# atneit/SCA-LDPC

Measured on AMD Instinct MI355X. Metric: edge_message_updates_per_s, higher is better.
Workload: dtype f32; 1 GPU; hqc128 H=[Hin|I] N=17669 W=50 R=4000 E=204000, batch 4096/GPU, 50 fixed iters, min_sum; batch_per_gpu=4096, iters=50, tile_group=0

## Files before the change

### sca-ldpc_amd/csrc/scaldpc_bp.hip

```cpp
#include "scaldpc_common.h"
#include "scaldpc_bp_sched.h"
#include "scaldpc_mc_law.h"
#include "scaldpc_trials.h"

#include <algorithm>
#include <cfloat>
#include <cmath>
#include <cstdlib>
#include <cstring>
#include <mutex>
#include <unordered_map>
#include <vector>

typedef unsigned long long u64;

using namespace scaldpc;

#include "scaldpc_bp_kernels.h"
#include "scaldpc_bp_ref64.h"

namespace scaldpc {
int launch_mc_hqc_outcome64(const McHqcLaw64 &law, unsigned long long *synd, double *plane, int R, int batch, int T, long first,
                            unsigned k0, unsigned k1, int *acc_flips, int *acc_cost, uint8_t *out_outcome, hipStream_t s);
int launch_gather_prior64(const double *src, int cols, const int *ids, double *dst, int T2, hipStream_t s);
// ... 604 lines not shown
    const dim3 grid(h->row_bk.blk[h->row_bk.nb], G), block(256);
    const bool test = ft && !first;
    if (method != SCALDPC_BP_MIN_SUM) {
        with_cap<16, 32, 64>(h->max_row_deg, [&](auto cap) {
            if (test)
                hipLaunchKernelGGL((k_check_tanh<cap, false, true, SharedPrior>), grid, block, 0, s, h->d_row_list, msg0, scr0, synd_g,
                                   done_g, skip_done, h->m, h->E, h->d_col_idx, h->d_prior, *ft);
            else
                with_first_prior(h, first, sp, [&](auto fst, auto P, auto prior) {
                    hipLaunchKernelGGL((k_check_tanh<cap, fst, false, decltype(P)>), grid, block, 0, s, h->d_row_list, msg0, scr0,
                                       synd_g, done_g, skip_done, h->m, h->E, h->d_col_idx, prior, FusedTest{});
                });
        });
    } else if (rec_form(h, method) && !first) {
        float *const rec0 = h->d_rec + (size_t)tile0 * rec_tile_floats(h->m);
        u64 *const mask0 = h->d_mask + (size_t)tile0 * h->E;
        const FusedTest ft0 = test ? *ft : FusedTest{};
        const float *const cprior = sp ? nullptr : h->d_prior;
        with_cap<16, 32, 64>(h->max_row_deg, [&](auto cap) {
            with_bool(boot, [&](auto bt) {
                with_bool(test, [&](auto par) {
                    hipLaunchKernelGGL((k_check_minsum_rec<cap, bt, par>), grid, block, 0, s, h->d_row_list, msg0, synd_g, done_g,
                                       skip_done, h->m, h->E, alpha, h->d_col_idx, rec0, mask0, h->d_csr_pos, cprior, ft0, stl);
                });
            });
        });
    } else if (h->max_row_deg <= ROW_CAP) {
        with_cap<16, 32, 64>(h->max_row_deg, [&](auto cap) {
            if (test)
                hipLaunchKernelGGL((k_check_minsum_x<cap, false, true, SharedPrior>), grid, block, 0, s, h->d_row_list, msg0, synd_g,
                                   done_g, skip_done, h->m, h->E, alpha, h->d_col_idx, h->d_prior, *ft);
            else
                with_first_prior(h, first, sp, [&](auto fst, auto P, auto prior) {
                    hipLaunchKernelGGL((k_check_minsum_x<cap, fst, false, decltype(P)>), grid, block, 0, s, h->d_row_list, msg0,
                                       synd_g, done_g, skip_done, h->m, h->E, alpha, h->d_col_idx, prior, FusedTest{});
                });
        });
    } else {
        with_first_prior(h, first, sp, [&](auto fst, auto P, auto prior) {
            hipLaunchKernelGGL((k_check_minsum<fst, decltype(P)>), dim3((h->m + 3) / 4, G), block, 0, s, h->d_row_ptr, msg0, synd_g,
                               done_g, skip_done, h->m, h->E, alpha, h->d_col_idx, prior);
        });
    }
    LAUNCH_CHECK();
    return 0;
}

bool first_fusable(const scaldpc_bp *h, int method)
{
    return h->kn.first_fused && fused_init(h, method) && h->E > 0 && h->max_row_deg <= 64 && h->max_col_deg <= 64 &&
           !h->hg_var.has_generic;
}

int ensure_first_table(scaldpc_bp *h, int method, float alpha1, hipStream_t s)
{
    if (h->first_valid && h->first_method == method && h->first_alpha == alpha1) return 0;
    h->first_valid = false;
    SC_TRY(grow(h->d_first_tab, (size_t)h->E + 128));
    Buf<u64> zero;
    Buf<float> tmp;
    SC_TRY(tmp.ensure((size_t)h->E));
    SC_TRY(zero.ensure((size_t)h->m + 1));
    hipError_t e = hipMemsetAsync(zero, 0, sizeof(u64) * ((size_t)h->m + 1), s);
    if (e == hipSuccess) e = hipMemsetAsync(h->d_first_tab, 0, sizeof(int2) * h->d_first_tab.cap(), s);
    if (e == hipSuccess) {
        with_method(method, [&](auto M) {
            hipLaunchKernelGGL((k_el_check<M, true, SharedPrior>), dim3((h->m + 3) / 4, 1), dim3(256), 0, s, h->d_row_ptr, h->d_col_idx,
                               h->d_prior, tmp, zero, zero + h->m, 0, h->m, h->E, alpha1, (const u64 *)nullptr, (int *)nullptr);
        });
        hipLaunchKernelGGL(k_first_tab, dim3((unsigned)((h->E + 255) / 256)), dim3(256), 0, s, h->d_csc_list, tmp, h->d_row_ptr, h->m,
                           h->E, h->d_first_tab);
        e = hipGetLastError();
    }
    if (e == hipSuccess) e = hipStreamSynchronize(s);
    if (e != hipSuccess) return fail(SCALDPC_EHIP, "first-message table: %s", hipGetErrorString(e));
    h->first_valid = true;
    h->first_method = method;
    h->first_alpha = alpha1;
    return 0;
}

int launch_var(scaldpc_bp *h, int G, float *post_g, u64 *hard_g, const u64 *done_g, int skip_done, int write_out,
               hipStream_t s, int tile0 = 0, const u64 *first_synd = nullptr, bool rec = false, bool light = false,
               const SoftPrior *sp = nullptr, bool final_pass = false, const Settle &stl = Settle{})
{
    float *const msg0 = h->d_msg + (size_t)tile0 * h->E * TW;
    float *const scr0 = h->d_scratch ? h->d_scratch + (size_t)tile0 * h->E * TW : nullptr;
    const int nblk = h->var_bk.blk[h->var_bk.nb];
    if (first_synd) {
        const int nrec = 4 * nblk;
        const dim3 grid2((unsigned)((nrec + 7) / 8), G);
        with_cap<16, 32, 64>(h->max_col_deg, [&](auto cap) {
            hipLaunchKernelGGL((k_var_first<cap>), grid2, dim3(256), 0, s, h->d_var_meta, h->d_csc_list, h->d_prior, msg0, post_g,
                               hard_g, done_g, skip_done, h->n, h->E, write_out, (const int2 *)h->d_first_tab, first_synd, h->m, nrec);
        });
    } else if (rec) {
        const int n1 = (h->var_bk.nb > 0 && h->var_bk.maxd[0] == 1) ? h->var_bk.blk[1] : 0;
        const bool slim = light && !write_out && n1 > 0 && n1 < nblk;
        const int nb_launch = slim ? nblk - n1 : nblk;
        const bool xm = G == 2 || G == 4 || G == 8;
        const dim3 gridr((unsigned)(xm ? (nb_launch + 7) / 8 * 8 : nb_launch), G);
        const int blk0 = slim && !h->var_reversed ? n1 : 0, xmap = xm ? nb_launch : 0;
        with_cap<16, 32>(h->max_col_deg, [&](auto cap) {
            with_prior(h, sp, [&](auto P, auto prior) {
                with_bool(final_pass && write_out, [&](auto fin) {
                    hipLaunchKernelGGL((k_var_rec<cap, decltype(P), fin>), gridr, dim3(256), 0, s, h->d_var_meta, h->d_var_rows,
                                       h->d_csc_list, h->d_csc_row, prior, msg0, h->d_rec + (size_t)tile0 * rec_tile_floats(h->m),
                                       h->d_mask + (size_t)tile0 * h->E, post_g, hard_g, done_g, skip_done, h->n, h->m, h->E,
                                       write_out, blk0, xmap, stl);
                });
            });
        });
    } else {
        with_cap<16, 32, 64>(h->max_col_deg, [&](auto cap) {
            with_prior(h, sp, [&](auto P, auto prior) {
                hipLaunchKernelGGL((k_var<cap, decltype(P)>), dim3(nblk, G), dim3(256), 0, s, h->d_var_meta, h->d_csc_list, prior, msg0,
                                   scr0, post_g, hard_g, done_g, skip_done, h->n, h->E, write_out);
            });
        });
    }
    LAUNCH_CHECK();
    return 0;
}

int launch_el_check(scaldpc_bp *h, int method, float alpha, int nb, const u64 *synd_g, const u64 *done_g,
                    int skip_done, hipStream_t s, bool first, const u64 *hard_g = nullptr, int *unsat_prev = nullptr,
                    const SoftPrior *sp = nullptr)
{
    with_method(method, [&](auto M) {
        with_first_prior(h, first, sp, [&](auto fst, auto P, auto prior) {
            hipLaunchKernelGGL((k_el_check<M, fst, decltype(P)>), dim3((h->m + 3) / 4, nb), dim3(256), 0, s, h->d_row_ptr,
                               h->d_col_idx, prior, h->d_emsg, synd_g, done_g, skip_done, h->m, h->E, alpha, hard_g, unsat_prev);
        });
    });
    LAUNCH_CHECK();
    return 0;
}

int launch_el_var(scaldpc_bp *h, int nb, float *post_g, u64 *hard_g, u64 *done_g, int skip_done, int write_out,
                  hipStream_t s, const int *unsat_prev = nullptr, int it_prev = 0, u64 *conv_g = nullptr,
                  int *iters_g = nullptr, int *remaining_prev = nullptr, const SoftPrior *sp = nullptr)
{
    const unsigned gx = (unsigned)(((h->el_waves + 3) / 4 + 7) / 8 * 8);
    with_prior(h, sp, [&](auto P, auto prior) {
        hipLaunchKernelGGL((k_el_var<decltype(P)>), dim3(gx, nb), dim3(256), 0, s, (const int2 *)h->d_el_slots, h->d_el_slot_col,
                           h->el_waves, prior, h->d_emsg, post_g, hard_g, done_g, skip_done, h->E, write_out, unsat_prev, it_prev,
                           conv_g, iters_g, remaining_prev);
    });
    LAUNCH_CHECK();
    return 0;
}

int launch_syndrome(const scaldpc_bp *h, const u64 *x, u64 *synd, int T, hipStream_t s)
{
    hipLaunchKernelGGL(k_parity<false>, dim3(parity_blocks(h->m), T), dim3(256), 0, s, h->d_row_ptr, h->d_col_idx, x, h->m, h->n,
                       synd, (u64 *)nullptr, (const u64 *)nullptr);
    LAUNCH_CHECK();
    return 0;
}

size_t small_lds_bytes(const scaldpc_bp *h) { return (size_t)2 * h->E * sizeof(float) + (size_t)2 * h->n + h->m + 64; }
size_t small_lds(const scaldpc_bp *h)
{
    const size_t lds = small_lds_bytes(h);
    const bool fits = h->E > 0 && lds <= 60 * 1024;
    return fits && h->kn.path != Knobs::STREAM && h->kn.path != Knobs::EDGE ? lds : 0;
}

template <bool PLANES>
int launch_small(scaldpc_bp *h, size_t lds, int method, int batch, const void *in, int input_kind, int max_iter, float alpha,
                 bool early, void *bits, float *llr, int *iters, void *conv, hipStream_t s, const SoftPrior *sp = nullptr)
{
    with_method(method, [&](auto M) {
        auto launch = [&](auto P, auto prior) {
            hipLaunchKernelGGL((k_bp_small<M, PLANES, decltype(P)>), dim3(batch), dim3(256), lds, s, h->d_row_ptr, h->d_col_idx,
                               h->d_col_ptr, h->d_csc_edge, prior, h->m, h->n, (int)h->E, in, input_kind, max_iter, alpha,
                               early ? 1 : 0, bits, llr, iters, conv);
        };
        with_prior(h, sp, launch);
    });
    LAUNCH_CHECK();
    return 0;
}

float alpha_for(float alpha, int it)
{
    return alpha == 0.0f ? (float)(1.0 - std::pow(2.0, -1.0 * it)) : alpha;
}

struct TileState {
    const u64 *synd;
    u64 *hard, *done, *conv, *unsat;
// ... 55 lines not shown
constexpr int MAX_LANES = SCHED_MAX_LANES;
int fixed_lanes(const scaldpc_bp *h, int g)
{
    if (h->E == 0) return 1;
    return lanes_of(h->kn.split, g);
}
int ensure_lanes(scaldpc_bp *h, int nl)
{
    for (int k = 1; k < nl; k++)
        if (!h->aux_stream[k]) {
            int dev = 0;
            SC_TRY(stream_acquire(&h->aux_stream[k], &dev));
            SC_HIP(hipEventCreateWithFlags(&h->ev_join[k], hipEventDisableTiming));
            SC_HIP(hipEventCreateWithFlags(&h->ev_phase[k], hipEventDisableTiming));
        }
    if (nl > 1 && !h->ev_join[0]) SC_HIP(hipEventCreateWithFlags(&h->ev_join[0], hipEventDisableTiming));
    return 0;
}
struct Lanes {
    scaldpc_bp *h;
    hipStream_t s;
    int n = 1;
    bool open = false;
    Lanes(scaldpc_bp *h_, hipStream_t s_) : h(h_), s(s_) {}
    Lanes(const Lanes &) = delete;
    Lanes &operator=(const Lanes &) = delete;
    ~Lanes() { if (open) (void)join(); }
    hipStream_t operator[](int k) const { return k ? h->aux_stream[k] : s; }
    int fork(int nl)
    {
        n = nl;
        open = nl > 1;
        if (!open) return 0;
        SC_HIP(hipEventRecord(h->ev_join[0], s));
        for (int k = 1; k < n; k++) SC_HIP(hipStreamWaitEvent(h->aux_stream[k], h->ev_join[0], 0));
        return 0;
    }
    int join()
    {
        for (int k = 1; k < n; k++) {
            SC_HIP(hipEventRecord(h->ev_join[k], h->aux_stream[k]));
            SC_HIP(hipStreamWaitEvent(s, h->ev_join[k], 0));
        }
        open = false;
        return 0;
    }
};


struct SettlePlan {
    unsigned *words = nullptr;
    int first_test = 0, horizon = 0;
};
int iterate_tiles(scaldpc_bp *h, Lanes &lanes, const TileState &st, int g0, int g, int max_iter, int method, float alpha,
                  bool early, int defer_after, bool *deferred, int real_codewords, PollState &ps, int chain,
                  const SettlePlan &sl = SettlePlan{})
{
    const hipStream_t s = lanes.s;
    const int skip = early ? 1 : 0;
    const int nl = fixed_lanes(h, g);
    SC_TRY(ensure_lanes(h, nl));
    int gs[MAX_LANES], t0[MAX_LANES];
    deal_tiles(g, nl, gs, t0);
    const int pw = parity_waves(h);
    const bool fused = fused_init(h, method);
    const bool soft = st.pprior != nullptr;
    if (h->E && !fused) {
        const SoftPrior spv = soft ? soft_prior(h, st, g0) : SoftPrior{};
        with_prior(h, soft ? &spv : nullptr, [&](auto P, auto prior) {
            hipLaunchKernelGGL((k_init_msg<decltype(P)>), dim3((unsigned)((h->E + 3) / 4), g), dim3(256), 0, s, h->d_col_idx,
                               h->d_msg.get(), h->E, prior);
        });
        LAUNCH_CHECK();
    }
    int *rem = h->d_remaining;
    if (early) SC_TRY(next_remaining_row(h, s, &rem, lanes.open));
    if (!(chain & 1)) SC_TRY(lanes.fork(nl));
    const bool first_fuse = first_fusable(h, method) && !soft;
    if (first_fuse) SC_TRY(ensure_first_table(h, method, alpha_for(alpha, 1), s));
    const bool ride = early && h->kn.fuse_test && check_can_test(h, method) && pw >= FT_WORDS;
    bool verdict_pending[MAX_LANES] = {};
    const bool recf = rec_form(h, method);
    bool rec_booted[MAX_LANES] = {};
    bool set_phase = true;
    const bool tracked = sl.words && recf && !early;
    const int K = tracked ? sl.horizon : 0, last_test = K ? K : max_iter;
    if (K) h->settle_saved += (long)nl * settle_launches_saved(K, max_iter);
    for (int it = 1; it <= max_iter; it++) {
        const bool last = it == max_iter;
        if (!settle_enqueued(it, K, max_iter)) continue;
        const bool no_check = (first_fuse && it == 1) || !settle_has_check(it, K, max_iter);
        const bool poll = poll_point(it, defer_after, ps);
        lanes.open = nl > 1;
        for (int k = 0; k < nl && !no_check; k++) {
            const int ta = g0 + t0[k];
            FusedTest ft{};
            if (verdict_pending[k]) {
                ft = FusedTest{st.hard + (size_t)ta * h->n, st.unsat + (size_t)ta * pw, st.done + ta, st.conv + ta,
                               st.iters + (size_t)ta * TW, rem + (it - 1), h->n, pw, it - 1, 1};
                verdict_pending[k] = false;
            }
            const SoftPrior spv = soft ? soft_prior(h, st, ta) : SoftPrior{};
            const bool first = fused && it == 1, boot = recf && !first && !rec_booted[k];
            if (boot) rec_booted[k] = true;
            Settle stc{};
            if (tracked)
                stc = Settle{sl.words + (size_t)ta * SETTLE_WORDS, settle_check_done(it, sl.first_test),
                             boot ? 0 : settle_check_mark(it, sl.first_test, last_test)};
            SC_TRY(launch_check(h, method, alpha_for(alpha, it), gs[k], st.synd + (size_t)ta * h->m, st.done + ta, skip, lanes[k],
                                first, t0[k], ft.hard ? &ft : nullptr, soft ? &spv : nullptr, boot, stc));
            if (set_phase && k + 1 < nl) {
                SC_HIP(hipEventRecord(h->ev_phase[k + 1], lanes[k]));
                SC_HIP(hipStreamWaitEvent(lanes[k + 1], h->ev_phase[k + 1], 0));
            }
        }
        if (!no_check) set_phase = false;
        if (!settle_has_var(it, K)) continue;
        for (int k = 0; k < nl; k++) {
            const int ta = g0 + t0[k];
            const SoftPrior spv = soft ? soft_prior(h, st, ta) : SoftPrior{};
            Settle stv{};
            if (tracked && !last)
                stv = Settle{sl.words + (size_t)ta * SETTLE_WORDS, settle_var_done(it, sl.first_test, last_test),
                             settle_var_mark(it, sl.first_test, last_test)};
            SC_TRY(launch_var(h, gs[k], st.post ? st.post + (size_t)ta * h->n * TW : nullptr, st.hard + (size_t)ta * h->n,
                              st.done + ta, skip, (early || last) ? 1 : 0, lanes[k], t0[k],
                              first_fuse && it == 1 ? st.synd + (size_t)ta * h->m : nullptr, it > 1 && recf, it > 1,
                              soft ? &spv : nullptr, last, stv));
            if (ride && !last && !poll) {
                verdict_pending[k] = true;
            } else if (early || last) {
                const dim3 grid(parity_blocks(h->m), gs[k]);
                if (pw >= FT_WORDS && h->kn.fuse_test) {
                    const FusedTest pf{st.hard + (size_t)ta * h->n, st.unsat + (size_t)ta * pw, st.done + ta, st.conv + ta,
                                       st.iters + (size_t)ta * TW, rem + it, h->n, pw, it, early ? 1 : 0};
                    hipLaunchKernelGGL(k_parity_fin_sharded, grid, dim3(256), 0, lanes[k], h->d_row_ptr, h->d_col_idx, h->m,
                                       st.synd + (size_t)ta * h->m, pf);
                } else
                    hipLaunchKernelGGL(k_parity_fin, grid, dim3(256), 0, lanes[k], h->d_row_ptr, h->d_col_idx,
                                       st.hard + (size_t)ta * h->n, h->m, h->n, st.synd + (size_t)ta * h->m,
                                       st.unsat + (size_t)ta * pw, pw, it, early ? 1 : 0, st.done + ta, st.conv + ta,
                                       st.iters + (size_t)ta * TW, rem + it);
                LAUNCH_CHECK();
            }
        }
        if (!early || last || !poll) continue;
        if (it == defer_after && stops_unseen(defer_after, max_iter, ps)) {
            note_unseen(ps);
            h->sched.w[SCHED_UNSEEN]++;
            *deferred = true;
            if (chain & 2) return 0;
            return lanes.join();
        }
        SC_TRY(lanes.join());
        SC_HIP(hipMemcpyAsync(h->h_remaining + it, rem + it, sizeof(int), hipMemcpyDeviceToHost, s));
        SC_HIP(hipStreamSynchronize(s));
        set_phase = true;
        h->sched.w[SCHED_POLLS]++;
        const PollVerdict v = after_poll(ps, it, defer_after, max_iter, h->h_remaining[it], real_codewords, g, el_limit(h, method));
        if (v == POLL_DONE) return 0;
        if (v == POLL_HAND_OVER) {
            *deferred = true;
            return 0;
        }
    }
    if (chain & 2) return 0;
    return lanes.join();
}

int ensure_level(scaldpc_bp *h, scaldpc_bp::Level &L, int T2)
{
    if (T2 <= L.cap_tiles) return 0;
    L.synd.reset(); L.hard.reset(); L.done.reset(); L.conv.reset(); L.unsat.reset();
    L.iters.reset(); L.ids.reset();
    L.cap_tiles = 0;
    SC_TRY(L.synd.ensure((size_t)T2 * h->m));
    SC_TRY(L.hard.ensure((size_t)T2 * h->n));
    SC_TRY(L.done.ensure((size_t)T2));
    SC_TRY(L.conv.ensure((size_t)T2));
    SC_TRY(L.unsat.ensure((size_t)T2 * parity_waves(h)));
    SC_TRY(L.iters.ensure((size_t)T2 * TW));
    SC_TRY(L.ids.ensure((size_t)T2 * TW));
    L.cap_tiles = T2;
    return 0;
}

int decode_level(scaldpc_bp *h, int lvl, const TileState &st, int batch, int T, int G, int max_iter, int method,
                 float alpha, bool early, bool want_post, hipStream_t s)
{
    const int lim = el_limit(h, method);
    const int el = (T == 1 && batch <= lim) ? batch : 0;
    const int Gl = std::min(G, T);
    if (el)
        SC_TRY(ensure_el(h, el));
    else
        SC_TRY(ensure_msg(h, Gl, method));
    if (lvl == 0) {
        h->last_group = el ? 0 : Gl;
        h->last_early = early;
    }
    h->stat_levels = lvl;
    if (el) {
        h->stat_el = el;
        return iterate_el(h, st, el, max_iter, method, alpha, early, s);
    }

    const int defer_after = defer_after_of(early, lvl, h->kn.compact_after, max_iter);
    SC_HIP(hipMemsetAsync(st.unsat, 0, sizeof(u64) * (size_t)T * parity_waves(h), s));
    std::vector<char> deferred_tile(T, 0);
    bool any = false;
    PollState poll;
// ... 1714 lines not shown
```

### sca-ldpc_amd/csrc/scaldpc_bp_kernels.h

```cpp
#pragma once
#include "scaldpc_logf.h"
#include "scaldpc_mc_law.h"
#include "scaldpc_philox.h"
#include "scaldpc_mc_draw.h"
#include "scaldpc_rec_pack.h"
#include "scaldpc_rec_trim.h"
#include <type_traits>

extern "C" __device__ int scaldpc_llvm_writelane(int src, int lane, int old) __asm("llvm.amdgcn.writelane.i32");

namespace {

__device__ __forceinline__ unsigned writelane(unsigned src, int lane, unsigned old)
{
    return (unsigned)scaldpc_llvm_writelane((int)src, lane, (int)old);
}

constexpr int TW = 64;
constexpr int MAXB = 8;
constexpr int ROW_CAP = 64;
#ifndef REC_CHUNK
#define REC_CHUNK 8
#endif

__device__ __forceinline__ int rfl(int x) { return __builtin_amdgcn_readfirstlane(x); }

struct SharedPrior {
    typedef const float *__restrict__ Arg;
    const float *prior;
    __device__ __forceinline__ float operator()(int v, int, int) const { return prior[v]; }
};
struct SoftPrior {
    typedef SoftPrior Arg;
    const float *prior;
    const float *plane;
    int first_col, cols;
    __device__ __forceinline__ float operator()(int v, int tl, int lane) const
    {
        const float *src = v >= first_col ? plane + ((size_t)tl * cols + (v - first_col)) * 64 + lane : prior + v;
        return *src;
    }
};

template <int CAP, class F>
__device__ __forceinline__ void for_exact_degree(int deg, F &&f)
{
#define XD(D)                                                        \
    case D:                                                          \
        if constexpr (D <= CAP) f(std::integral_constant<int, D>{}); \
        break;
#define XD8(D) XD(D) XD(D + 1) XD(D + 2) XD(D + 3) XD(D + 4) XD(D + 5) XD(D + 6) XD(D + 7)
    switch (deg) {
        XD(1) XD(2) XD(3) XD(4) XD(5) XD(6) XD(7)
        XD8(8) XD8(16) XD8(24) XD8(32) XD8(40) XD8(48) XD8(56)
        XD(64)
        default: break;
    }
#undef XD8
#undef XD
}

__global__ __launch_bounds__(256) void k_pack_bits(const uint8_t *__restrict__ in, int len, int batch,
                                                   u64 *__restrict__ out)
{
    const int lane = threadIdx.x & 63;
    const int x0 = (blockIdx.x * 4 + (threadIdx.x >> 6)) * 16;
    const int t = blockIdx.y;
    if (x0 >= len) return;
    const long b = (long)t * TW + lane;
    const uint8_t *p = in + (size_t)(b < batch ? b : 0) * len + x0;
    const int nx = min(16, len - x0);
    for (int j = 0; j < nx; j++) {
        const int bit = (b < batch) ? (p[j] & 1) : 0;
        const u64 w = __ballot(bit);
        if (lane == 0) out[(size_t)t * len + x0 + j] = w;
    }
}

__global__ __launch_bounds__(256) void k_unpack_bits(const u64 *__restrict__ hard, const u64 *__restrict__ recv,
                                                     int n, int batch, uint8_t *__restrict__ out)
{
    const int v = blockIdx.x * 256 + threadIdx.x;
    const int t = blockIdx.y;
    if (v >= n) return;
    u64 w = hard[(size_t)t * n + v];
    if (recv) w ^= recv[(size_t)t * n + v];
    const int nb = min(TW, batch - t * TW);
    for (int c = 0; c < nb; c++) out[(size_t)(t * TW + c) * n + v] = (uint8_t)((w >> c) & 1);
}

__global__ __launch_bounds__(256) void k_unpack_llr(const float *__restrict__ post, int n, int batch,
                                                    float *__restrict__ out)
{
    __shared__ float tile[64][65];
    const int t = blockIdx.y, v0 = blockIdx.x * 64;
    const int lane = threadIdx.x & 63, w = threadIdx.x >> 6;
    for (int j = w; j < 64; j += 4)
        if (v0 + j < n) tile[j][lane] = post[((size_t)t * n + v0 + j) * TW + lane];
    __syncthreads();
    for (int c = w; c < 64; c += 4) {
        const long b = (long)t * TW + c;
        if (b < batch && v0 + lane < n) out[(size_t)b * n + v0 + lane] = tile[lane][c];
    }
}

__global__ __launch_bounds__(256) void k_soft_convert(const float *__restrict__ probs, int cols, int batch,
                                                      float *__restrict__ plane, u64 *__restrict__ bad)
{
    __shared__ float tile[64][65];
    const int t = blockIdx.y, j0 = blockIdx.x * 64;
    const int lane = threadIdx.x & 63, w = threadIdx.x >> 6;
    for (int c = w; c < 64; c += 4) {
        const long b = (long)t * TW + c;
        float l = 0.0f;
        if (b < batch && j0 + lane < cols) {
            const size_t i = (size_t)b * cols + j0 + lane;
            const float p = probs[i];
            if (p >= 0.0f && p <= 1.0f)
                l = scaldpc::glibc_logf((1.0f - p) / p);
            else
                atomicMin(bad, (u64)i);
        }
        tile[c][lane] = l;
    }
    __syncthreads();
    for (int j = w; j < 64; j += 4)
        if (j0 + j < cols) plane[((size_t)t * cols + j0 + j) * TW + lane] = tile[lane][j];
}

__global__ __launch_bounds__(64) void k_unpack_state(const u64 *__restrict__ conv_bits, const int *__restrict__ iters,
                                                     int batch, int *__restrict__ out_iters,
                                                     uint8_t *__restrict__ out_conv)
{
    const int t = blockIdx.x, c = threadIdx.x;
    const long b = (long)t * TW + c;
    if (b >= batch) return;
    if (out_iters) out_iters[b] = iters[b];
    if (out_conv) out_conv[b] = (uint8_t)((conv_bits[t] >> c) & 1);
}

__global__ __launch_bounds__(256) void k_small_prepare(const uint8_t *__restrict__ in, int len, int batch,
                                                       u64 *__restrict__ planes, int n, u64 *__restrict__ hard,
                                                       int max_iter, u64 *__restrict__ done, u64 *__restrict__ conv,
                                                       int *__restrict__ iters, int *__restrict__ remaining, int nrem,
                                                       int *__restrict__ el_unsat, int nun)
{
    const int lane = threadIdx.x & 63;
    const int x0 = (blockIdx.x * 4 + (threadIdx.x >> 6)) * 16;
    const uint8_t *p = in + (size_t)(lane < batch ? lane : 0) * len;
    for (int j = 0; j < 16; j++) {
        const int x = x0 + j;
        if (x < len) {
            const u64 w = __ballot(lane < batch && (p[x] & 1));
            if (lane == 0) planes[x] = w;
        }
        if (x < n && lane == 0) hard[x] = 0;
    }
    if (blockIdx.x == 0) {
        if (threadIdx.x < 64) {
// ... 1103 lines not shown
        for (int k = VAR_INLINE; k < D; k++) rw[k] = cr1[k];
    }
    u64 sg = 0;
    if ((int)lane < D) sg = sgn_col[lane];
    const int slo = (int)(unsigned)sg, shi = (int)(unsigned)(sg >> 32);
    float mm[D], pp[D];
    unsigned ab[D];
#pragma unroll
    for (int k = 0; k < D; k++) ab[k] = sbase_b(arg_base + (size_t)rec_row_of(rfl(rw[k])) * TW)[lane];
    const unsigned off1 = lane * 4u, off2 = off1 + rec2_off;
#pragma unroll
    for (int k = 0; k < D; k++) {
        const unsigned off = ab[k] == (unsigned)rec_index_of(rfl(rw[k])) ? off2 : off1;
        mm[k] = *(const gfloat *)((const gbyte *)sbase(rec_base + (size_t)rec_row_of(rfl(rw[k])) * TW) + off);
    }
#pragma unroll
    for (int k = 0; k < D; k++) {
        const u64 ng = ((u64)(unsigned)__builtin_amdgcn_readlane(shi, k) << 32) | (unsigned)__builtin_amdgcn_readlane(slo, k);
        mm[k] = __builtin_amdgcn_inverse_ballot_w64(ng) ? -mm[k] : mm[k];
    }
    if constexpr (LAST) {
        float sum = pr;
#pragma unroll
        for (int k = 0; k < D; k++) sum += mm[k];
        return sum;
    }
    {
        const int4 *rec4 = (const int4 *)rc;
        const int4 a = rec4[1], b = rec4[2], c = rec4[3], e = rec4[4];
        const int in16[16] = {a.x, a.y, a.z, a.w, b.x, b.y, b.z, b.w, c.x, c.y, c.z, c.w, e.x, e.y, e.z, e.w};
#pragma unroll
        for (int k = 0; k < D && k < VAR_INLINE; k++) eid[k] = in16[k];
    }
    float temp = pr;
#pragma unroll
    for (int k = 0; k < D; k++) {
        pp[k] = temp;
        temp += mm[k];
    }
#pragma unroll
    for (int k = VAR_INLINE; k < D; k++) eid[k] = ce1[k];
    float suf = 0.0f;
    unsigned nlo = 0, nhi = 0;
#pragma unroll
    for (int k = D - 1; k >= 0; k--) {
        gfloat *q = sbase(tile_base + (size_t)rfl(eid[k]) * TW) + lane;
        const float out = pp[k] + suf;
        __hip_atomic_store(q, out, __ATOMIC_RELAXED, __HIP_MEMORY_SCOPE_AGENT);
        const u64 nm = __ballot(out <= 0.0f);
        nlo = writelane((unsigned)nm, k, nlo);
        nhi = writelane((unsigned)(nm >> 32), k, nhi);
        suf += mm[k];
    }
    if ((int)lane < D) sgn_col[lane] = ((u64)nhi << 32) | nlo;
    if (mark_word) {
        const unsigned dlo = (nlo ^ (unsigned)slo) & (unsigned)real, dhi = (nhi ^ (unsigned)shi) & (unsigned)(real >> 32);
        if (__ballot((int)lane < D && (dlo | dhi) != 0) != 0 && lane == 0) *mark_word = mark;
    }
    return temp;
}

template <int CAP, class P, bool LAST = false>
__global__ __launch_bounds__(256) void k_var_rec(const int *__restrict__ list, const int *__restrict__ var_rows,
                                                 const int *__restrict__ csc_edge, const int *__restrict__ csc_row,
                                                 typename P::Arg prior_arg, float *msg, const float *__restrict__ rec,
                                                 u64 *sgn, float *__restrict__ post,
                                                 u64 *__restrict__ hard, const u64 *__restrict__ done, int skip_done, int n, int m,
                                                 long E, int write_out, int blk0, int xmap, Settle stl = Settle{})
{
    const P prior{prior_arg};
    const unsigned lane = threadIdx.x & 63u;
    int tl = blockIdx.y, bx = blockIdx.x;
    if (xmap) {
        const unsigned G = gridDim.y, L = blockIdx.y * gridDim.x + blockIdx.x, xcd = L & 7u, slot = L >> 3;
        tl = (int)(xcd % G);
        bx = (int)(slot * (8u / G) + xcd / G);
        if (bx >= xmap) return;
    }
    const int ri = rfl((bx + blk0) * 4 + (int)(threadIdx.x >> 6));
    const int *rc = list + (size_t)ri * VAR_REC;
    const u64 dn = done[tl];
    if (skip_done && dn == ~0ull) return;
    unsigned *mark_word = nullptr;
    if (!LAST && stl.words) {
        unsigned *w = stl.words + (size_t)tl * SETTLE_WORDS;
        if (settle_frozen(w, stl.done)) return;
        if (stl.mark) mark_word = w + ((unsigned)bx & (SETTLE_SHARDS - 1));
    }
    const int v = rc[0];
    if (v < 0) return;
    const int cb = rc[1];
    const int d = rc[2];
    float *tb = msg + (size_t)tl * E * TW;
    const float *rb = rec + (size_t)tl * rec_tile_floats(m);
    const unsigned char *ab = (const unsigned char *)(rb + rec_arg_off(m));
    u64 *st = sgn + (size_t)tl * E;
    const int *ce = csc_edge + cb, *cr = csc_row + cb;
    const int4 *w4 = (const int4 *)(var_rows + (size_t)ri * VAR_INLINE);
    const float pr = prior(v, tl, (int)lane);
    float L = pr;
    const unsigned r2 = (unsigned)m * (TW * (unsigned)sizeof(float));
#define VR(D)                                                                                                \
    case D:                                                                                                  \
        if constexpr (D <= CAP)                                                                              \
            L = var_col_rec<D, LAST>(tb, rb, r2, ab, st + cb, lane, rc, w4, ce, cr, pr, mark_word, (unsigned)stl.mark, ~dn); \
        break;
#define VR8(D) VR(D) VR(D + 1) VR(D + 2) VR(D + 3) VR(D + 4) VR(D + 5) VR(D + 6) VR(D + 7)
    switch (d) {
        VR(1) VR(2) VR(3) VR(4) VR(5) VR(6) VR(7)
        VR8(8) VR8(16) VR8(24) VR(32)
        default: break;
    }
#undef VR8
#undef VR
    if (write_out) {
        const u64 hb = __ballot(L <= 0.0f);
        const size_t hi = (size_t)tl * n + v;
        if (lane == 0) hard[hi] = (hard[hi] & dn) | (hb & ~dn);
        if (post && !((dn >> lane) & 1)) post[hi * TW + lane] = L;
    }
}
__device__ __forceinline__ float wave_min_f(float v)
{
#pragma unroll
    for (int off = 32; off >= 1; off >>= 1) v = fminf(v, __shfl_xor(v, off));
    return v;
}
__device__ __forceinline__ float readlane_f(float v, int l)
{
    return __int_as_float(__builtin_amdgcn_readlane(__float_as_int(v), l));
}

template <int METHOD, bool FIRST, class P>
__global__ __launch_bounds__(256) void k_el_check(const int *__restrict__ row_ptr, const int *__restrict__ col_idx,
                                                  typename P::Arg prior_arg, float *emsg,
                                                  const u64 *__restrict__ synd, const u64 *__restrict__ done,
                                                  int skip_done, int m, long E, float alpha,
                                                  const u64 *__restrict__ hard, int *__restrict__ unsat_prev)
{
    const P prior{prior_arg};
    const int lane = threadIdx.x & 63;
    int r = blockIdx.x * 4 + (threadIdx.x >> 6);
    if (r >= m) return;
    r = rfl(r);
    const int c = blockIdx.y;
    if (skip_done && ((done[0] >> c) & 1)) return;
    const int e0 = rfl(row_ptr[r]);
    const int deg = rfl(row_ptr[r + 1]) - e0;
    const bool act = lane < deg;
    const unsigned sbit = (unsigned)(synd[r] >> c) & 1u;
    if (unsat_prev) {
        const unsigned hb = act ? (unsigned)(hard[col_idx[e0 + lane]] >> c) & 1u : 0u;
        if ((((unsigned)__popcll(__ballot(hb != 0u)) & 1u) ^ sbit) && lane == 0) unsat_prev[c] = 1;
    }
    if (deg == 0) return;
    float *p = emsg + (size_t)c * E + e0 + lane;
    float x = 0.0f;
    if (act) x = FIRST ? prior(col_idx[e0 + lane], 0, c) : *p;
    if (METHOD == SCALDPC_BP_MIN_SUM) {
        const float a = act ? fminf(fabsf(x), FLT_MAX) : FLT_MAX;
        const bool ng = act && x <= 0.0f;
        const unsigned par = sbit ^ ((unsigned)__popcll(__ballot(ng)) & 1u);
        const float m1 = wave_min_f(a);
        const int ix = __ffsll((long long)__ballot(act && a == m1)) - 1;
        const float m2 = wave_min_f(lane == ix ? FLT_MAX : a);
        if (act) *p = ((lane == ix) ? m2 : m1) * ((par ^ (unsigned)ng) ? -alpha : alpha);
    } else {
        const unsigned xb = act ? __float_as_uint(x) : 0u;
        const float u = act ? tanh_compl(fabsf(x)) : 0.0f;
        const unsigned par = sbit ^ ((unsigned)__popcll(__ballot((xb >> 31) != 0u)) & 1u);
        float pre = 0.0f, suf = 0.0f;
#pragma unroll 4
        for (int t = 0; t < deg; t++) {
            const float nv = compl_step(pre, readlane_f(u, t));
            pre = (t < lane) ? nv : pre;
        }
#pragma unroll 4
        for (int t = deg - 1; t >= 0; t--) {
            const float nv = compl_step(suf, readlane_f(u, t));
            suf = (t > lane) ? nv : suf;
        }
        const float Lm = llr_from_compl(compl_step(pre, suf));
        const unsigned sg = ((par << 31) ^ xb) & 0x80000000u;
        if (act) *p = __uint_as_float(__float_as_uint(Lm) ^ sg);
    }
}
template <class P>
__device__ __forceinline__ void el_var_body(const int2 *__restrict__ slots, const int *__restrict__ slot_col,
                                            int nwaves, P prior, float *emsg,
                                            float *__restrict__ post, u64 *__restrict__ hard,
                                            u64 *done, int skip_done, long E, int write_out,
                                            const int *__restrict__ unsat_prev, int it_prev, u64 *conv,
                                            int *__restrict__ iters, int *__restrict__ remaining_prev)
{
    const int lane = threadIdx.x & 63;
    int w = blockIdx.x * 4 + (threadIdx.x >> 6);
    if (w >= nwaves) return;
    w = rfl(w);
    const int c = blockIdx.y;
    const bool frozen = (done[0] >> c) & 1;
    if (skip_done && frozen) return;
// ... 221 lines not shown
```

### sca-ldpc_amd/csrc/scaldpc_bp_sched.h

```cpp
#pragma once

#include <cstdint>

namespace scaldpc {

constexpr int SCHED_TW = 64;
constexpr int SCHED_MAX_LANES = 4;
constexpr int SCHED_MAX_LEVELS = 3;
constexpr int REM_SLOTS = 512;

constexpr int SPEC_PERIOD = 16;
constexpr int POLL_EVERY = 4;
struct PollState {
    int hint = 1, streak = 0, since_poll = 0;
};
inline bool poll_point(int it, int defer_after, const PollState &ps)
{
    return (it % POLL_EVERY == 0 || it == 1 || it == defer_after) && it >= ps.hint;
}
inline bool stops_unseen(int defer_after, int max_iter, const PollState &ps)
{
    return defer_after > 0 && 2 * defer_after < max_iter && ps.streak >= 2 && ps.since_poll < SPEC_PERIOD - 1 &&
           poll_point(defer_after, defer_after, ps);
}
inline bool runs_unseen(int defer_after, int max_iter, const PollState &ps)
{
    if (!stops_unseen(defer_after, max_iter, ps)) return false;
    for (int it = 1; it < defer_after; it++)
        if (poll_point(it, defer_after, ps)) return false;
    return true;
}
inline void note_unseen(PollState &ps) { ps.since_poll++; }

inline int lanes_of(int split, int g)
{
    const int nl = split < g ? split : g;
    return nl < 1 ? 1 : nl > SCHED_MAX_LANES ? SCHED_MAX_LANES : nl;
}
inline void deal_tiles(int g, int nl, int *gs, int *t0)
{
    for (int k = 0, t = 0; k < nl; k++) {
        gs[k] = g / nl + (k < g % nl ? 1 : 0);
        t0[k] = t;
        t += gs[k];
    }
}

inline int defer_after_of(bool early, int lvl, int compact_after, int max_iter)
{
    int defer_after = 0;
    if (early && lvl < SCHED_MAX_LEVELS) {
        defer_after = 4;
        if (compact_after >= 0) defer_after = compact_after;
        if (max_iter <= 2 * defer_after) defer_after = 0;
    }
    return defer_after;
}

enum PollVerdict { POLL_DONE = 0, POLL_HAND_OVER = 1, POLL_GO_ON = 2 };
inline PollVerdict after_poll(PollState &ps, int it, int defer_after, int max_iter, int left, int real, int g, int el_lim)
{
    if (left == 0) return POLL_DONE;
    if (left >= real) ps.hint = ps.hint > it + 1 ? ps.hint : it + 1;
    const bool shrinks = (left + SCHED_TW - 1) / SCHED_TW < g || left <= el_lim;
    if (defer_after > 0 && it >= defer_after && 2 * it < max_iter && 2 * left <= real && shrinks) {
        ps.streak = (it == defer_after && 8 * left <= real) ? ps.streak + 1 : 0;
        ps.since_poll = 0;
        return POLL_HAND_OVER;
    }
    if (it >= defer_after) ps.streak = 0;
    return POLL_GO_ON;
}

inline int ring_rows_wanted(int T, int G)
{
    const int gg = G > 1 ? G : 1;
    const int groups = (T + gg - 1) / gg;
    const int want = 2 * groups + 8;
    return want < REM_SLOTS ? want : REM_SLOTS;
}
struct RemRing {
    int slot = 0, rows = 0;
};
inline int ring_take(RemRing &r, bool *clears)
{
    *clears = r.slot >= r.rows;
    if (*clears) r.slot = 1;
    return r.slot++;
}

inline int chain_bits(bool early, bool lanes2, bool full, bool first, bool next_full, bool lanes_open, int defer_after,
                      int max_iter, const PollState &ps, const RemRing &ring)
{
    int chain = 0;
    if (!lanes2 || !full) return 0;
    if (!early) {
        if (!first) chain |= 1;
        if (next_full) chain |= 2;
    } else if (runs_unseen(defer_after, max_iter, ps)) {
        PollState nxt = ps;
        note_unseen(nxt);
        if (lanes_open) chain |= 1;
        if (next_full && runs_unseen(defer_after, max_iter, nxt) && ring.slot + 2 < ring.rows) chain |= 2;
    }
    return chain;
}

enum SchedWord {
    SCHED_GROUPS = 0,
    SCHED_HANDED = 4,
    SCHED_POLLS = 7,
    SCHED_UNSEEN = 8,
    SCHED_CONTINUED = 9,
    SCHED_LEFT_OPEN = 10,
    SCHED_FIXED_CHAINED = 11,
    SCHED_CLEARS = 12,
    SCHED_OPEN_AT_CLEAR = 13,
    SCHED_RING_ROWS = 14,
    SCHED_EL_POLLS = 15,
    SCHED_RING_TAKES = 16,
    SCHED_WORDS = 17
};
struct SchedCounters {
    int64_t w[SCHED_WORDS] = {};
    bool ring_cleared = false;
    void reset() { *this = SchedCounters{}; }
    void note_take(bool clears, bool lanes_open)
    {
        w[SCHED_RING_TAKES]++;
        if (!clears) return;
        if (ring_cleared) w[SCHED_CLEARS]++;
        if (lanes_open) w[SCHED_OPEN_AT_CLEAR]++;
        ring_cleared = true;
    }
    void note_group(int lvl, bool early, int chain)
    {
        w[SCHED_GROUPS + lvl]++;
        if (early) {
            if (chain & 1) w[SCHED_CONTINUED]++;
            if (chain & 2) w[SCHED_LEFT_OPEN]++;
        } else if (chain & 1)
            w[SCHED_FIXED_CHAINED]++;
    }
};

constexpr int SETTLE_FIRST = 3;
inline int settle_first_test(int alpha_from)
{
    const int t = alpha_from + 1;
    return t < SETTLE_FIRST ? SETTLE_FIRST : t;
}
inline int settle_check_done(int it, int first_test) { return it - 1 >= first_test ? it - 1 : 0; }
inline int settle_check_mark(int it, int first_test, int last_test) { return it >= first_test && it <= last_test ? it : 0; }
inline int settle_var_done(int it, int first_test, int last_test) { return it >= first_test && it <= last_test ? it : 0; }
inline int settle_var_mark(int it, int first_test, int last_test) { return settle_check_mark(it + 1, first_test, last_test); }
inline int settle_frozen_at(int latest, int first_test, int last_test)
{
    if (last_test < first_test || latest >= last_test) return 0;
    return latest + 1 > first_test ? latest + 1 : first_test;
}
inline bool settle_horizon_usable(int K, int first_test, int max_iter) { return K >= first_test && K + 1 < max_iter; }
inline bool settle_enqueued(int it, int K, int max_iter) { return !(K && it > K && it < max_iter); }
inline bool settle_has_check(int it, int K, int max_iter) { return !(K && it == max_iter); }
inline bool settle_has_var(int it, int K) { return !(K && it == K); }
inline int settle_launches_saved(int K, int max_iter) { return 2 * (max_iter - K); }
inline int settle_next_horizon(int tiles, int frozen, int max_frozen_at, int rerun, int max_iter)
{
    if (tiles <= 0 || max_frozen_at <= 0) return 0;
    if (8 * rerun > tiles) return 0;
    const int K = max_frozen_at + 2;
    if (8 * frozen < 7 * tiles) return 0;
    if (2 * K >= max_iter) return 0;
    return K;
}

inline int settle_mode(int knob, bool identity_block) { return knob >= 0 ? knob : identity_block ? 2 : 0; }

inline bool el_poll_point(int ip) { return (ip >= 3 && ip <= 6) || (ip > 6 && ip <= 16 && ip % 2 == 0) || (ip > 16 && ip % 16 == 0); }

}
```

Baseline: 8124 billion directed edge-message updates/s.

## Skip frozen-tile var work in last pass by keeping hard bits live; vectorize bit packing

When settle tracking is active and no posterior output is requested, intermediate k_var_rec passes now write hard decisions. This lets the final pass skip higher-degree variables in tiles already frozen, which removes redundant work in the last iteration. k_pack_bits now loads 16 bytes with aligned word reads and assigns one output word per lane, replacing the byte-by-byte loop with a lane-0 store. The hard write also avoids a read-modify-write when no lanes are done. It adds hard-bit writes on every tracked iteration, and correctness depends on the stored hard bits staying valid for frozen tiles.

```diff
diff --git a/profiles/minsum_settle_passes/lane_account.py b/profiles/minsum_settle_passes/lane_account.py
--- /dev/null
+++ b/profiles/minsum_settle_passes/lane_account.py
@@ -0,0 +1,55 @@
+import collections
+import csv
+import re
+import sys
+
+
+def kind(name):
+    m = re.search(r"(k_\w+)(<[^>]*>)?", name)
+    if not m:
+        return name.split("(")[0]
+    k, t = m.group(1), m.group(2) or ""
+    if k == "k_var_rec":
+        return "k_var_rec<last>" if t.rstrip(">").endswith("true") else "k_var_rec"
+    if k == "k_check_minsum_rec":
+        return "k_check_minsum_rec<BOOT>" if t.split(",")[1].strip() == "true" else "k_check_minsum_rec"
+    return k
+
+
+def main():
+    rows = list(csv.DictReader(open(sys.argv[1])))
+    ev = sorted(((int(r["Start_Timestamp"]), int(r["End_Timestamp"]), r["Stream_Id"], r["Queue_Id"], kind(r["Kernel_Name"]))
+                 for r in rows))
+    first = max(i for i, e in enumerate(ev) if e[4] == "k_pack_bits")
+    ev = ev[first:]
+    t0, t1 = ev[0][0], max(e[1] for e in ev)
+    print(f"step: {len(ev)} dispatches, {(t1 - t0) / 1e3:.1f} us from the start of k_pack_bits to the end of the last kernel")
+    lanes = collections.defaultdict(list)
+    for e in ev:
+        lanes[(e[2], e[3])].append(e)
+    for (stream, queue), es in sorted(lanes.items()):
+        busy = sum(e[1] - e[0] for e in es)
+        print(f"\nstream {stream} (queue {queue}): {len(es)} dispatches, busy {busy / 1e3:.1f} us, "
+              f"first start +{(es[0][0] - t0) / 1e3:.1f} us, last end +{(es[-1][1] - t0) / 1e3:.1f} us")
+        by = collections.defaultdict(list)
+        for e in es:
+            by[e[4]].append((e[1] - e[0]) / 1e3)
+        for k, v in sorted(by.items(), key=lambda kv: -sum(kv[1])):
+            short = sum(1 for x in v if x < 8.0)
+            print(f"  {k:28s} {len(v):4d} launches, {sum(v):8.1f} us in all, mean {sum(v) / len(v):6.1f}, of them {short} under 8 us")
+        gaps = collections.defaultdict(list)
+        for a, b in zip(es, es[1:]):
+            gaps[(a[4], b[4])].append((b[0] - a[1]) / 1e3)
+        idle = sum(sum(v) for v in gaps.values())
+        print(f"  idle between consecutive launches: {idle:.1f} us in all")
+        for (a, b), v in sorted(gaps.items(), key=lambda kv: -sum(kv[1])):
+            if sum(v) >= 5.0:
+                print(f"    {a} -> {b}: {len(v)} gaps, {sum(v):.1f} us in all, mean {sum(v) / len(v):.2f}, max {max(v):.1f}")
+        waits = [(b[0] - a[1]) / 1e3 for a, b in zip(es, es[1:]) if a[4] == "k_var_first" and b[4].startswith("k_check_minsum_rec")]
+        if waits:
+            print(f"  wait between k_var_first and the group's first check pass: {len(waits)} groups, mean {sum(waits) / len(waits):.1f} us, "
+                  f"{sum(waits):.1f} us in all")
+
+
+if __name__ == "__main__":
+    main()
diff --git a/sca-ldpc_amd/csrc/scaldpc_bp.hip b/sca-ldpc_amd/csrc/scaldpc_bp.hip
--- a/sca-ldpc_amd/csrc/scaldpc_bp.hip
+++ b/sca-ldpc_amd/csrc/scaldpc_bp.hip
@@ -710,7 +710,7 @@
 
 int launch_var(scaldpc_bp *h, int G, float *post_g, u64 *hard_g, const u64 *done_g, int skip_done, int write_out,
                hipStream_t s, int tile0 = 0, const u64 *first_synd = nullptr, bool rec = false, bool light = false,
-               const SoftPrior *sp = nullptr, bool final_pass = false, const Settle &stl = Settle{})
+               const SoftPrior *sp = nullptr, bool final_pass = false, const Settle &stl = Settle{}, bool keep_hard = false)
 {
     float *const msg0 = h->d_msg + (size_t)tile0 * h->E * TW;
     float *const scr0 = h->d_scratch ? h->d_scratch + (size_t)tile0 * h->E * TW : nullptr;
@@ -735,7 +735,7 @@
                     hipLaunchKernelGGL((k_var_rec<cap, decltype(P), fin>), gridr, dim3(256), 0, s, h->d_var_meta, h->d_var_rows,
                                        h->d_csc_list, h->d_csc_row, prior, msg0, h->d_rec + (size_t)tile0 * rec_tile_floats(h->m),
                                        h->d_mask + (size_t)tile0 * h->E, post_g, hard_g, done_g, skip_done, h->n, h->m, h->E,
-                                       write_out, blk0, xmap, stl);
+                                       (write_out || keep_hard) ? 1 : 0, blk0, xmap, stl);
                 });
             });
         });
@@ -957,10 +957,11 @@
     bool verdict_pending[MAX_LANES] = {};
     const bool recf = rec_form(h, method);
     bool rec_booted[MAX_LANES] = {};
-    bool set_phase = true;
     const bool tracked = sl.words && recf && !early;
     const int K = tracked ? sl.horizon : 0, last_test = K ? K : max_iter;
+    bool set_phase = phase_reestablished(chain, K, max_iter);
     if (K) h->settle_saved += (long)nl * settle_launches_saved(K, max_iter);
+    const bool keep_hard = tracked && st.post == nullptr;
     for (int it = 1; it <= max_iter; it++) {
         const bool last = it == max_iter;
         if (!settle_enqueued(it, K, max_iter)) continue;
@@ -998,10 +999,12 @@
             if (tracked && !last)
                 stv = Settle{sl.words + (size_t)ta * SETTLE_WORDS, settle_var_done(it, sl.first_test, last_test),
                              settle_var_mark(it, sl.first_test, last_test)};
+            else if (keep_hard)
+                stv = Settle{sl.words + (size_t)ta * SETTLE_WORDS, last_test, 0};
             SC_TRY(launch_var(h, gs[k], st.post ? st.post + (size_t)ta * h->n * TW : nullptr, st.hard + (size_t)ta * h->n,
                               st.done + ta, skip, (early || last) ? 1 : 0, lanes[k], t0[k],
                               first_fuse && it == 1 ? st.synd + (size_t)ta * h->m : nullptr, it > 1 && recf, it > 1,
-                              soft ? &spv : nullptr, last, stv));
+                              soft ? &spv : nullptr, last, stv, keep_hard && !last));
             if (ride && !last && !poll) {
                 verdict_pending[k] = true;
             } else if (early || last) {
diff --git a/sca-ldpc_amd/csrc/scaldpc_bp_kernels.h b/sca-ldpc_amd/csrc/scaldpc_bp_kernels.h
--- a/sca-ldpc_amd/csrc/scaldpc_bp_kernels.h
+++ b/sca-ldpc_amd/csrc/scaldpc_bp_kernels.h
@@ -68,13 +68,32 @@
     const int t = blockIdx.y;
     if (x0 >= len) return;
     const long b = (long)t * TW + lane;
-    const uint8_t *p = in + (size_t)(b < batch ? b : 0) * len + x0;
     const int nx = min(16, len - x0);
-    for (int j = 0; j < nx; j++) {
-        const int bit = (b < batch) ? (p[j] & 1) : 0;
-        const u64 w = __ballot(bit);
-        if (lane == 0) out[(size_t)t * len + x0 + j] = w;
-    }
+    unsigned w[4] = {0u, 0u, 0u, 0u};
+    if (b < batch) {
+        const uint8_t *p = in + (size_t)b * len + x0;
+        const size_t lo = (size_t)in, hi = lo + (size_t)batch * len, pa = (size_t)p;
+        const unsigned mis = (unsigned)(pa & 3u);
+        const size_t a = pa - mis;
+        if (a >= lo && a + 20 <= hi) {
+            const unsigned *q = (const unsigned *)a;
+            unsigned d[5];
+#pragma unroll
+            for (int i = 0; i < 5; i++) d[i] = q[i];
+#pragma unroll
+            for (int i = 0; i < 4; i++) w[i] = (unsigned)(((((u64)d[i + 1]) << 32) | d[i]) >> (8u * mis));
+        } else {
+            for (int j = 0; j < nx; j++) w[j >> 2] |= (unsigned)p[j] << (8 * (j & 3));
+        }
+    }
+    u64 mine = 0;
+#pragma unroll
+    for (int j = 0; j < 16; j++) {
+        if (j >= nx) break;
+        const u64 word = __ballot((w[j >> 2] >> (8 * (j & 3))) & 1u);
+        if (lane == j) mine = word;
+    }
+    if (lane < nx) out[(size_t)t * len + x0 + lane] = mine;
 }
 
 __global__ __launch_bounds__(256) void k_unpack_bits(const u64 *__restrict__ hard, const u64 *__restrict__ recv,
@@ -1344,15 +1363,22 @@
     const u64 dn = done[tl];
     if (skip_done && dn == ~0ull) return;
     unsigned *mark_word = nullptr;
-    if (!LAST && stl.words) {
+    bool decided = false;
+    if (stl.words) {
         unsigned *w = stl.words + (size_t)tl * SETTLE_WORDS;
-        if (settle_frozen(w, stl.done)) return;
-        if (stl.mark) mark_word = w + ((unsigned)bx & (SETTLE_SHARDS - 1));
+        const bool frozen = settle_frozen(w, stl.done);
+        if constexpr (LAST)
+            decided = frozen;
+        else {
+            if (frozen) return;
+            if (stl.mark) mark_word = w + ((unsigned)bx & (SETTLE_SHARDS - 1));
+        }
     }
     const int v = rc[0];
     if (v < 0) return;
     const int cb = rc[1];
     const int d = rc[2];
+    if (LAST && decided && d > 1) return;
     float *tb = msg + (size_t)tl * E * TW;
     const float *rb = rec + (size_t)tl * rec_tile_floats(m);
     const unsigned char *ab = (const unsigned char *)(rb + rec_arg_off(m));
@@ -1378,7 +1404,10 @@
     if (write_out) {
         const u64 hb = __ballot(L <= 0.0f);
         const size_t hi = (size_t)tl * n + v;
-        if (lane == 0) hard[hi] = (hard[hi] & dn) | (hb & ~dn);
+        if (dn == 0) {
+            if (lane == 0) hard[hi] = hb;
+        } else if (lane == 0)
+            hard[hi] = (hard[hi] & dn) | (hb & ~dn);
         if (post && !((dn >> lane) & 1)) post[hi * TW + lane] = L;
     }
 }
diff --git a/sca-ldpc_amd/csrc/scaldpc_bp_sched.h b/sca-ldpc_amd/csrc/scaldpc_bp_sched.h
--- a/sca-ldpc_amd/csrc/scaldpc_bp_sched.h
+++ b/sca-ldpc_amd/csrc/scaldpc_bp_sched.h
@@ -106,6 +106,14 @@
     return chain;
 }
 
+inline bool phase_reestablished(int chain, int horizon, int max_iter)
+{
+    (void)chain;
+    (void)horizon;
+    (void)max_iter;
+    return true;
+}
+
 enum SchedWord {
     SCHED_GROUPS = 0,
     SCHED_HANDED = 4,
```

Measured after the change: 8379 billion directed edge-message updates/s (median of 6 runs). 1.03x the previous value.
